# importZL/semantic_segmentation

Hardware: AMD Instinct MI355X
Metric: images/sec (fwd+bwd) U-Net 256x256 bs=32 per GPU (higher is better)
Workload: dtype f16; 1 GPU; unet.UNet(1,2) 256x256 fwd+bwd, CE+Dice loss, batch 32/GPU (BASELINE configs[1]); global_batch=32, parallelism=dp1, dice=per-rank

## Files before the change

### include/gsseg.h

```cpp
#ifndef GSSEG_H
#define GSSEG_H

#include <stdint.h>

#ifdef __cplusplus
extern "C" {
#endif

#define GS_ABI_VERSION 52

enum GsDtype { GS_F16 = 0, GS_BF16 = 1 };
enum GsStatus { GS_OK = 0, GS_EINVAL = -1, GS_ELAUNCH = -2, GS_EUNSUPPORTED = -3 };
enum GsAct { GS_ACT_NONE = 0, GS_ACT_RELU = 1, GS_ACT_LEAKY02 = 2, GS_ACT_TANH = 3 };

#define GS_MAX_TAPS 64

typedef struct GsConvGeom {
    int32_t N, IH, IW, Cin, in_pix_stride, in_coff;
    int32_t OHg, OWg, Cout;
    int32_t OH, OW, out_pix_stride, out_coff;
    int32_t isy, isx, osy, osx, ooy, oox;
    int32_t ntaps;
    int32_t tap_dy[GS_MAX_TAPS], tap_dx[GS_MAX_TAPS];
    int32_t tap_w[GS_MAX_TAPS];
    int32_t Dg, Din, Dout, isz, osz, ooz;
    int32_t tap_dz[GS_MAX_TAPS];
} GsConvGeom;

const char* gs_last_error(void);
int gs_abi_version(void);

int gs_conv_igemm_mtiles(const GsConvGeom* g);
int64_t gs_conv_igemm_workspace_floats(void);
int gs_conv_igemm(const GsConvGeom* g, const void* x, const void* w, void* y, const float* bias,
                  float* bn_partials, int act, int dtype, float* splitk_ws, int64_t splitk_ws_floats, void* stream);
int gs_conv_igemm_batch(int n, const GsConvGeom* const* g, const void* x, const void* const* w, void* y, const float* bias,
                        float* const* bn_partials, int act, int dtype, float* splitk_ws, int64_t splitk_ws_floats,
                        void* stream);

int gs_upconv2x2_fwd(const void* x, const void* w, const float* bias, void* y, int N, int D, int IH, int IW, int Cin,
                     int in_pix_stride, int in_coff, int Cout, int Dout, int OH, int OW, int out_pix_stride,
                     int out_coff, int ooz, int ooy, int oox, int act, int dtype, void* stream);

int gs_upconv2x2_dgrad(const void* dy, const void* wd, void* dx, int N, int IH, int IW, int Cin, int Cout, int OH, int OW,
                       int dy_pix_stride, int dy_coff, int ooy, int oox, int dx_pix_stride, int dx_coff, int dtype,
                       void* stream);

int gs_conv3x3_mtiles(int N, int H, int W, int Cout);
int gs_conv3x3_stat_rows(int N, int H, int W, int Cin, int Cout, int pair);
int gs_conv3x3_set_kernel_form(int form);
int gs_set_persistent_grid(int blocks);
int gs_get_persistent_grid(void);
int gs_conv3x3(const void* x, const void* w, void* y, const float* bias, float* bn_partials, int N, int H, int W,
               int Cin, int in_pix_stride, int in_coff, int Cout, int out_pix_stride, int out_coff,
               const int32_t* tap_dy, const int32_t* tap_dx, int act, int dtype, void* stream);

int gs_conv3x3_wgrad(const void* x, const void* dy, float* dw, int N, int H, int W, int Cin, int in_pix_stride,
                     int in_coff, int Cout, int out_pix_stride, int out_coff, int dtype, void* stream);

int gs_conv_wgrad(const GsConvGeom* g, const void* x, const void* dy, float* dw, int dtype, void* stream);
int gs_conv_wgrad_single_pass(const GsConvGeom* g);
int gs_conv_wgrad_assign(const GsConvGeom* g, const void* x, const void* dy, float* dw, int dtype, void* stream);
int gs_conv_wgrad_parts(const GsConvGeom* g);
int64_t gs_conv_wgrad_ws_floats(const GsConvGeom* g);
int gs_conv_wgrad_slabs(const GsConvGeom* g, const void* x, const void* dy, float* ws, int dtype, void* stream);
int gs_conv_wgrad_slabs_batch(int n, const GsConvGeom* const* g, const void* x, const void* dy, float* ws, int dtype,
                              void* stream);

int gs_conv_smallcin_mtiles(int N, int OH, int OW);
int gs_conv_smallcin_fwd(const float* x, const float* w, const float* bias, void* y, float* bn_partials,
                         int N, int Cin, int IH, int IW, int Cout, int OH, int OW, int k, int stride, int pad,
                         int act, int dtype, void* stream);
int64_t gs_conv_direct_wgrad_ws_floats(int N, int OH, int OW, int Cin, int Cout, int k);

int gs_stem_stats(const float* x, const float* w, float* bn_partials, float* tap_sums, int N, int H, int W, void* stream);
int gs_stem_fwd_bn(const float* x, const float* w, const float* bn_scale, const float* bn_shift, int act, void* z, int N,
                   int H, int W, int dtype, void* stream);
int gs_stem_bwd_tiles(int N, int H, int W);
int gs_stem_bwd_onepass(const float* x, const void* z, const void* dz, int dz_stride, int dz_coff, int act,
                        float* s1_partials, float* ws, int N, int H, int W, int dtype, void* stream);
int gs_stem_bwd_finalize(const float* ws, const float* s1_partials, const float* tap_sums, const float* w,
                         const float* scale, const float* mean, const float* invstd, int train_stats, float gscale, float* dw,
                         float* dgamma, float* dbeta, int N, int H, int W, void* stream);

int gs_stem_bn_bwd_wgrad(const void* y, const void* dz, int dz_stride, int dz_coff, const float* x, const float* scale,
                         const float* shift, const float* mean, const float* invstd, const float* c1, const float* c2,
                         int act, float* dw, float* ws, int N, int H, int W, float gscale, int dtype, void* stream);

int gs_conv_smallcin_wgrad(const float* x, const void* dy, float* dw, float* ws, int N, int Cin, int IH, int IW,
                           int Cout, int OH, int OW, int k, int stride, int pad, float gscale, int dtype, void* stream);
int gs_conv_smallcin_dgrad(const void* dy, const float* w, float* dx, int N, int Cin, int IH, int IW, int Cout,
// ... 252 lines not shown
```

### semantic_segmentation_amd/_lib.py

```python
from __future__ import annotations

import ctypes
import os
import subprocess
from ctypes import POINTER, c_char_p, c_double, c_float, c_int, c_int32, c_int64, c_void_p

_HERE = os.path.dirname(os.path.abspath(__file__))
LIB_PATH = os.environ.get("GSSEG_LIB", os.path.join(_HERE, "libgsseg_hip.so"))
CSRC = os.path.join(_HERE, "csrc")

GS_F16, GS_BF16 = 0, 1
ACT_NONE, ACT_RELU, ACT_LEAKY02, ACT_TANH = 0, 1, 2, 3
GS_MAX_TAPS = 64
ABI_VERSION = 52


class GsConvGeom(ctypes.Structure):
    _fields_ = [(n, c_int32) for n in (
        "N", "IH", "IW", "Cin", "in_pix_stride", "in_coff", "OHg", "OWg", "Cout", "OH", "OW",
        "out_pix_stride", "out_coff", "isy", "isx", "osy", "osx", "ooy", "oox", "ntaps")] + [
        ("tap_dy", c_int32 * GS_MAX_TAPS), ("tap_dx", c_int32 * GS_MAX_TAPS), ("tap_w", c_int32 * GS_MAX_TAPS)] + [
        (n, c_int32) for n in ("Dg", "Din", "Dout", "isz", "osz", "ooz")] + [("tap_dz", c_int32 * GS_MAX_TAPS)]


class GsPackDesc(ctypes.Structure):
    _fields_ = [("w", c_void_p), ("w_fwd", c_void_p), ("w_dgrad", c_void_p)] + [
        (n, c_int32) for n in ("Cout", "Cin", "taps", "transposed")]


GS_SEG_MAX = 4


class GsSegPackDesc(ctypes.Structure):
    _fields_ = [("w", c_void_p), ("pack", c_void_p)] + [(n, c_int32) for n in ("Cout", "Cin", "taps", "transposed", "nseg")] + [
        ("kind", c_int32 * GS_SEG_MAX), ("ci0", c_int32 * GS_SEG_MAX), ("len", c_int32 * GS_SEG_MAX)]


class GsQ8PackDesc(ctypes.Structure):
    _fields_ = [("w", c_void_p), ("pack", c_void_p), ("wexp", c_void_p)] + [(n, c_int32) for n in ("Cout", "Cin", "taps")]


_P, _F = c_void_p, c_void_p
PROTOTYPES = {
    "gs_last_error": (c_char_p, []),
    "gs_abi_version": (c_int, []),
    "gs_conv_igemm_mtiles": (c_int, [POINTER(GsConvGeom)]),
    "gs_conv3x3_stat_rows": (c_int, [c_int] * 6),
    "gs_upconv2x2_wgrad_parts": (c_int, [c_int] * 5),
    "gs_upconv2x2_wgrad_ws_floats": (c_int64, [c_int] * 5),
    "gs_upconv2x2_wgrad_slabs": (c_int, [_P, _P, _F] + [c_int] * 14 + [c_void_p]),
    "gs_set_persistent_grid": (c_int, [c_int]),
    "gs_get_persistent_grid": (c_int, []),
    "gs_conv_igemm": (c_int, [POINTER(GsConvGeom), _P, _P, _P, _F, _F, c_int, c_int, _F, c_int64, c_void_p]),
    "gs_conv_igemm_workspace_floats": (c_int64, []),
    "gs_conv_igemm_batch": (c_int, [c_int, POINTER(POINTER(GsConvGeom)), _P, POINTER(c_void_p), _P, _F, POINTER(c_void_p),
                                    c_int, c_int, _F, c_int64, c_void_p]),
    "gs_upconv2x2_fwd": (c_int, [_P, _P, _F, _P] + [c_int] * 18 + [c_void_p]),
    "gs_upconv2x2_dgrad": (c_int, [c_void_p, c_void_p, c_void_p] + [c_int] * 14 + [c_void_p]),
    "gs_conv3x3_mtiles": (c_int, [c_int, c_int, c_int, c_int]),
    "gs_conv3x3_set_kernel_form": (c_int, [c_int]),
    "gs_conv3d_3x3x3_mtiles": (c_int, [c_int] * 5),
    "gs_conv3d_3x3x3": (c_int, [_P, _P, _P, _F, _F] + [c_int] * 10 + [POINTER(c_int32)] * 3 + [c_int, c_int, c_void_p]),
    "gs_conv3d_3x3x3_wgrad_ws_floats": (c_int64, [c_int] * 6),
    "gs_conv3d_3x3x3_wgrad_parts": (c_int, [c_int] * 6),
    "gs_conv3d_3x3x3_wgrad_slabs": (c_int, [_P, _P, _F] + [c_int] * 11 + [c_void_p]),
    "gs_conv3d_3x3x3_wgrad": (c_int, [_P, _P, _F] + [c_int] * 11 + [c_void_p]),
    "gs_upsample2x_bilinear_fwd": (c_int, [_P, _P] + [c_int] * 13 + [c_void_p]),
    "gs_upsample2x_bilinear_bwd": (c_int, [_P, _P] + [c_int] * 13 + [c_void_p]),
    "gs_affine_warp": (c_int, [_F, _F, _F, c_int, c_int, c_int, c_int, c_float, c_void_p]),
    "gs_optim_chunk_elems": (c_int, []),
    "gs_optim_rmsprop": (c_int, [_P] * 7 + [c_int] + [c_float] * 6 + [c_void_p]),
    "gs_optim_adam": (c_int, [_P] * 7 + [c_int, _P] + [c_float] * 5 + [c_void_p]),
    "gs_conv3x3": (c_int, [_P, _P, _P, _F, _F] + [c_int] * 9 + [POINTER(c_int32), POINTER(c_int32), c_int, c_int, c_void_p]),
    "gs_conv3x3_wgrad": (c_int, [_P, _P, _F] + [c_int] * 10 + [c_void_p]),
    "gs_conv3x3_wgrad_ws_floats": (c_int64, [c_int] * 5),
    "gs_conv3x3_wgrad_parts": (c_int, [c_int] * 5),
    "gs_conv3x3_wgrad_slabs": (c_int, [_P, _P, _F] + [c_int] * 10 + [c_void_p]),
    "gs_wgrad_reduce_unpack": (c_int, [_F, c_int, _F, c_int, c_int, c_int, c_int, c_float, c_void_p]),
    "gs_conv_wgrad": (c_int, [POINTER(GsConvGeom), _P, _P, _F, c_int, c_void_p]),
    "gs_conv_wgrad_assign": (c_int, [POINTER(GsConvGeom), _P, _P, _F, c_int, c_void_p]),
    "gs_conv_wgrad_single_pass": (c_int, [POINTER(GsConvGeom)]),
    "gs_conv_wgrad_parts": (c_int, [POINTER(GsConvGeom)]),
    "gs_conv_wgrad_ws_floats": (c_int64, [POINTER(GsConvGeom)]),
    "gs_conv_wgrad_slabs": (c_int, [POINTER(GsConvGeom), _P, _P, _F, c_int, c_void_p]),
    "gs_conv_wgrad_slabs_batch": (c_int, [c_int, POINTER(POINTER(GsConvGeom)), _P, _P, _F, c_int, c_void_p]),
    "gs_conv_smallcin_mtiles": (c_int, [c_int, c_int, c_int]),
    "gs_conv_smallcin_fwd": (c_int, [_F, _F, _F, _P, _F] + [c_int] * 12 + [c_void_p]),
    "gs_conv_direct_wgrad_ws_floats": (c_int64, [c_int] * 6),
    "gs_conv_smallcin_wgrad": (c_int, [_F, _P, _F, _F] + [c_int] * 10 + [c_float, c_int, c_void_p]),
    "gs_conv_smallcin_dgrad": (c_int, [_P, _F, _F] + [c_int] * 10 + [c_float, c_int, c_void_p]),
    "gs_conv_smallcout_fwd": (c_int, [_P, _F, _F, _F] + [c_int] * 11 + [c_void_p]),
    "gs_conv_smallcout_bwd": (c_int, [_P, _F, _F, _P, _F, _F, _F] + [c_int] * 10 + [c_float, c_int, c_void_p]),
    "gs_bn_partials_floats": (c_int64, [c_int, c_int]),
    "gs_bn_finalize": (c_int, [_F, c_int, c_int, c_double, _F, _F, _F, _F, c_float, c_float, _F, _F, _F, _F, c_void_p]),
    "gs_bn_eval_coeffs": (c_int, [c_int, _F, _F, _F, _F, c_float, _F, _F, _F, _F, c_void_p]),
    "gs_bn_act_apply": (c_int, [_P, _F, _F, c_int, _P, c_int, c_int, _P, _P, c_float] + [c_int] * 5 + [c_void_p]),
    "gs_bn_bwd_tiles": (c_int, [c_int, c_int, c_int]),
    "gs_bn_bwd_tiles_used": (c_int, [c_int, c_int, c_int, c_int]),
    "gs_bn_act_bwd_reduce": (c_int, [_P, _P, c_int, c_int, _P, _P, c_int, _P, c_float, _F, _F, _F, _F, c_int, _F]
                             + [c_int] * 5 + [c_void_p]),
    "gs_bn_bwd_coeffs": (c_int, [_F, c_int, c_int, c_double, c_float, _F, _F, _F, _F, c_void_p]),
    "gs_bn_act_bwd_apply": (c_int, [_P, _P, c_int, c_int, _P, _P, c_int, _P, c_float, _F, _F, _F, _F, _F, _F, c_int,
                                    c_int, _P]
                            + [c_int] * 5 + [c_void_p]),
    "gs_maxpool3d_fwd": (c_int, [_P, c_int, c_int, _P] + [c_int] * 6 + [c_void_p]),
    "gs_maxpool2x2_fwd": (c_int, [_P, c_int, c_int, _P] + [c_int] * 5 + [c_void_p]),
    "gs_maxpool2x2_fwd_pair": (c_int, [_P, _P, c_int, _P, _P, c_int] + [c_int] * 5 + [c_void_p]),
# ... 126 lines not shown
```

### semantic_segmentation_amd/csrc/wgrad3x3.hip

```cpp
#include <stdlib.h>

#include "common.hpp"

namespace {

struct W3Args {
    const unsigned short* x;
    const unsigned short* dy;
    float* dw;
    int N, H, W, Cin, in_stride, in_coff, Cout, out_stride, out_coff;
    int tiles_x, tiles_y, npatches, ncob, ncib, ksplit, pps;
    int D, dz;
    int64_t slab_stride;
};

constexpr int W3_LDR = 96;
constexpr int W3_BM = 128;

template <int DT, int TW>
__global__ __launch_bounds__(256, 2) void wgrad3x3_kernel(const W3Args a) {
    typedef typename Elem<DT>::V8 V8;
    constexpr int TH = W3_BM / TW;
    constexpr int HWD = TW + 2, HHT = TH + 2, HP = HWD * HHT;
    constexpr int DY_EL = W3_BM * W3_LDR, H_EL = HP * W3_LDR;
    constexpr int HCH = (HP * 8 + 255) / 256;
    constexpr int TWS = (TW == 32) ? 5 : 4;
    constexpr unsigned OOB = 0xFFFFFFFFu;
    __shared__ __attribute__((aligned(16))) unsigned short smem[DY_EL + H_EL];
    unsigned short* dyt = smem;
    unsigned short* halo = smem + DY_EL;

    const int t = threadIdx.x, lane = t & 63, wave = t >> 6;
    const int wm = wave >> 1, wn = wave & 1;
// ... 97 lines not shown
                const int hrow = (py + tap / 3) * HWD + px0 + tap % 3;
                const V8 bf = tr_read8<DT>(b_base + hrow * W3_LDR, b_base + (hrow + 4) * W3_LDR);
                acc[tap] = Elem<DT>::mfma32(af, bf, acc[tap]);
            }
        }
    }

    const int l31 = lane & 31, h = lane >> 5;
    const int ci = ci0 + wn * 32 + l31;
    if (ci < a.Cin) {
#pragma unroll
        for (int tap = 0; tap < 9; ++tap)
#pragma unroll
            for (int r = 0; r < 16; ++r) {
                const int co = co0 + wm * 32 + (r & 3) + 8 * (r >> 2) + 4 * h;
                if (co < a.Cout) {
                    float* q = a.dw + ((int64_t)tap * a.Cout + co) * a.Cin + ci;
                    if (a.slab_stride > 0) q[(int64_t)ks * a.slab_stride] = acc[tap][r];
                    else atomicAdd(q, acc[tap][r]);
                }
            }
    }
}


__device__ __forceinline__ void w3_dma_piece16(const __amdgpu_buffer_rsrc_t& rs, unsigned char* dst, unsigned voff) {
    const unsigned lds_addr = (unsigned)(size_t)(LDS_AS void*)dst;
    unsigned keep;
    asm volatile("s_mov_b32 %0, m0\n\ts_mov_b32 m0, %1\n\ts_nop 0\n\tbuffer_load_dwordx4 %2, %3, 0 offen lds\n\ts_mov_b32 m0, %0"
                 : "=&s"(keep) : "s"(lds_addr), "v"(voff), "s"(rs) : "memory");
}
__device__ __forceinline__ void w3_opaque(unsigned& x) { asm volatile("" : "+v"(x)); }

template <int DT>
__global__ __launch_bounds__(512, 1) void wgrad3x3_dma_kernel(const W3Args a) {
    typedef typename Elem<DT>::V8 V8;
    constexpr int TW = 32, TH = 8, TWS = 5, BM = 256;
    constexpr int HWD = TW + 2, HHT = TH + 2, HP = HWD * HHT;
    static_assert(BM / 8 == 4 * 8, "32 dY pieces: four per wave");
    constexpr int HJ = 6;
    constexpr int HPC = (HP + 7) / 8;
    constexpr int DY_B = BM * 128, HALO_B = (HPC + 1) * 1024;
    constexpr int HALO_OFF = 2 * DY_B;
    constexpr unsigned VOOB = 0x80000000u;
    static_assert(HPC + 1 <= HJ * 8 && 2 * (DY_B + HALO_B) <= 160 * 1024, "LDS budget");
    static_assert(4 * 9 * 16 * 64 * 4 <= 2 * (DY_B + HALO_B), "final in-block reduction overlays the stage buffers");
    __shared__ __attribute__((aligned(1024))) unsigned char smem[2 * (DY_B + HALO_B)];

    const int t = threadIdx.x, lane = t & 63;
    const int wave = __builtin_amdgcn_readfirstlane(t >> 6);
    const int grp = wave >> 2;
    const int wm = (wave >> 1) & 1, wn = wave & 1;
    int bid;
    {
        const int nwg = gridDim.x, q = nwg >> 3, r = nwg & 7, xcd = blockIdx.x & 7;
        bid = ((xcd < r) ? xcd * (q + 1) : r * (q + 1) + (xcd - r) * q) + (blockIdx.x >> 3);
    }
    const int cob = bid % a.ncob; bid /= a.ncob;
    const int cib = bid % a.ncib; bid /= a.ncib;
    const int ks = bid;
    const int co0 = cob * 64, ci0 = cib * 64;
    const int p_begin = ks * a.pps;
    const int p_end = min(a.npatches, p_begin + a.pps);
    if (p_begin >= p_end) return;

    const unsigned x_img_bytes = (unsigned)a.H * a.W * a.in_stride * 2u;
    const unsigned dy_img_bytes = (unsigned)a.H * a.W * a.out_stride * 2u;
// ... 64 lines not shown

    f32x16 acc[9];
#pragma unroll
    for (int i = 0; i < 9; ++i)
#pragma unroll
        for (int r = 0; r < 16; ++r) acc[i][r] = 0.f;

    const int G = lane >> 4, q = (lane & 15) >> 2, pp = lane & 3;
    const int krow = 8 * (G >> 1) + q;
    const int chn = 16 * (G & 1) + 4 * pp;
    unsigned a_base0 = (unsigned)((grp * 16 + krow) * 128 + (((wm ^ ((q >> 1) & 1)) * 32 + chn) * 2));
    unsigned b_base0[4];
#pragma unroll
    for (int c4 = 0; c4 < 4; ++c4)
        b_base0[c4] = (unsigned)(HALO_OFF + (grp * 16 + krow) * 128 + (((wn ^ (((c4 + q) >> 1) & 1)) * 32 + chn) * 2));

    {
        const Pf f0 = prep_patch(true);
#pragma unroll
        for (int k = 0; k < 4 + HJ; ++k) issue_piece(f0, k, 0u);
    }
    for (int patch = p_begin; patch < p_end; ++patch) {
        asm volatile("s_waitcnt vmcnt(0)" ::: "memory");
        __builtin_amdgcn_s_barrier();
        asm volatile("" ::: "memory");
        const unsigned buf = (unsigned)(patch - p_begin) & 1u;
        const bool more = patch + 1 < p_end;
        const Pf pf = prep_patch(more);
        unsigned ab = a_base0 + buf * DY_B, bb[4];
#pragma unroll
        for (int c4 = 0; c4 < 4; ++c4) { bb[c4] = b_base0[c4] + buf * HALO_B; w3_opaque(bb[c4]); }
        w3_opaque(ab);
        const LDS_AS unsigned char* lds = (const LDS_AS unsigned char*)smem;
        constexpr int PD = 3;
        V8 afr[2], bfr[PD + 1];
        auto load_a = [&](int s, V8& dst) __attribute__((always_inline)) {
            dst = tr_read8<DT>((const LDS_AS unsigned short*)(lds + ab + s * 32 * 128),
                               (const LDS_AS unsigned short*)(lds + ab + (s * 32 + 4) * 128));
        };
        auto load_b = [&](int step, V8& dst) __attribute__((always_inline)) {
            const int s = step / 9, tap = step - 9 * s;
            const int C = (s + tap / 3) * HWD + tap % 3;
            dst = tr_read8<DT>((const LDS_AS unsigned short*)(lds + bb[C & 3] + C * 128),
                               (const LDS_AS unsigned short*)(lds + bb[C & 3] + (C + 4) * 128));
        };
        load_a(0, afr[0]);
#pragma unroll
        for (int i = 0; i < PD; ++i) load_b(i, bfr[i]);
#pragma unroll
        for (int step = 0; step < 72; ++step) {
            const int s = step / 9, tap = step - 9 * s;
            if (step + PD < 72) load_b(step + PD, bfr[(step + PD) % (PD + 1)]);
            if (tap == 4 && s + 1 < 8) load_a(s + 1, afr[(s + 1) & 1]);
#if !defined(GS_W3_ABLATE) || GS_W3_ABLATE != 1
            if (s < 4 && (tap == 1 || tap == 4 || tap == 7) && 3 * s + tap / 3 < 4 + HJ) issue_piece(pf, 3 * s + tap / 3, buf ^ 1u);
#endif
#if !defined(GS_W3_ABLATE) || GS_W3_ABLATE != 2
            acc[tap] = Elem<DT>::mfma32(afr[s & 1], bfr[step % (PD + 1)], acc[tap]);
#endif
            __builtin_amdgcn_sched_group_barrier(0x008, 1, 0);
            __builtin_amdgcn_sched_group_barrier(0x100, 4, 0);
            __builtin_amdgcn_sched_barrier(0);
        }
    }
    asm volatile("s_waitcnt vmcnt(0)" ::: "memory");
    __syncthreads();
    float* xch = reinterpret_cast<float*>(smem) + (wave & 3) * (9 * 16 * 64) + lane;
    if (grp == 1) {
#pragma unroll
        for (int tap = 0; tap < 9; ++tap)
#pragma unroll
            for (int r = 0; r < 16; ++r) xch[(tap * 16 + r) * 64] = acc[tap][r];
    }
    __syncthreads();
    if (grp == 1) return;
    const int l31 = lane & 31, h = lane >> 5;
    const int ci = ci0 + wn * 32 + l31;
#pragma unroll
    for (int tap = 0; tap < 9; ++tap)
#pragma unroll
        for (int r = 0; r < 16; ++r) {
            const float v = acc[tap][r] + xch[(tap * 16 + r) * 64];
            const int co = co0 + wm * 32 + (r & 3) + 8 * (r >> 2) + 4 * h;
            if (ci < a.Cin && co < a.Cout) {
                float* qd = a.dw + ((int64_t)tap * a.Cout + co) * a.Cin + ci;
                if (a.slab_stride > 0) qd[(int64_t)ks * a.slab_stride] = v;
                else atomicAdd(qd, v);
            }
        }
}

template <int DT>
__global__ __launch_bounds__(512, 1) void wgrad3x3_dma128_kernel(const W3Args a) {
    typedef typename Elem<DT>::V8 V8;
    constexpr int TW = 32, TH = 4, TWS = 5, BM = 128;
    constexpr int HWD = TW + 2, HHT = TH + 2, HP = HWD * HHT;
    constexpr int DJ = 4;
    constexpr int HPC = (HP + 7) / 8;
    constexpr int HJ = 4;
    constexpr int IMG_B = BM * 128;
    constexpr int DY_B = 2 * IMG_B, HALO_B = (HPC + 1) * 1024;
    constexpr int HALO_OFF = 2 * DY_B;
    constexpr unsigned VOOB = 0x80000000u;
    static_assert(HPC + 1 <= HJ * 8 && 2 * (DY_B + HALO_B) <= 160 * 1024, "LDS budget");
    __shared__ __attribute__((aligned(1024))) unsigned char smem[2 * (DY_B + HALO_B)];

    const int t = threadIdx.x, lane = t & 63;
    const int wave = __builtin_amdgcn_readfirstlane(t >> 6);
    const int wmm = wave >> 1, wn = wave & 1;
    int bid;
    {
        const int nwg = gridDim.x, q = nwg >> 3, r = nwg & 7, xcd = blockIdx.x & 7;
        bid = ((xcd < r) ? xcd * (q + 1) : r * (q + 1) + (xcd - r) * q) + (blockIdx.x >> 3);
    }
    const int cob = bid % a.ncob; bid /= a.ncob;
    const int cib = bid % a.ncib; bid /= a.ncib;
    const int ks = bid;
    const int co0 = cob * 128, ci0 = cib * 64;
    const int p_begin = ks * a.pps;
    const int p_end = min(a.npatches, p_begin + a.pps);
    if (p_begin >= p_end) return;

    const unsigned x_img_bytes = (unsigned)a.H * a.W * a.in_stride * 2u;
    const unsigned dy_img_bytes = (unsigned)a.H * a.W * a.out_stride * 2u;
    const int drow = lane >> 3;
// ... 67 lines not shown

    f32x16 acc[9];
#pragma unroll
    for (int i = 0; i < 9; ++i)
#pragma unroll
        for (int r = 0; r < 16; ++r) acc[i][r] = 0.f;

    const int G = lane >> 4, q = (lane & 15) >> 2, pp = lane & 3;
    const int krow = 8 * (G >> 1) + q;
    const int chn = 16 * (G & 1) + 4 * pp;
    unsigned a_base0 = (unsigned)((wmm >> 1) * IMG_B + krow * 128 + ((((wmm & 1) ^ ((q >> 1) & 1)) * 32 + chn) * 2));
    unsigned b_base0[4];
#pragma unroll
    for (int c4 = 0; c4 < 4; ++c4)
        b_base0[c4] = (unsigned)(HALO_OFF + krow * 128 + (((wn ^ (((c4 + q) >> 1) & 1)) * 32 + chn) * 2));

    {
        const Pf f0 = prep_patch(true);
#pragma unroll
        for (int k = 0; k < DJ + HJ; ++k) issue_piece(f0, k, 0u);
    }
    for (int patch = p_begin; patch < p_end; ++patch) {
        asm volatile("s_waitcnt vmcnt(0)" ::: "memory");
        __builtin_amdgcn_s_barrier();
        asm volatile("" ::: "memory");
        const unsigned buf = (unsigned)(patch - p_begin) & 1u;
        const bool more = patch + 1 < p_end;
        const Pf pf = prep_patch(more);
        unsigned ab = a_base0 + buf * DY_B, bb[4];
#pragma unroll
        for (int c4 = 0; c4 < 4; ++c4) { bb[c4] = b_base0[c4] + buf * HALO_B; w3_opaque(bb[c4]); }
        w3_opaque(ab);
        const LDS_AS unsigned char* lds = (const LDS_AS unsigned char*)smem;
        constexpr int PD = 3;
        V8 afr[2], bfr[PD + 1];
        auto load_a = [&](int sg, V8& dst) __attribute__((always_inline)) {
            dst = tr_read8<DT>((const LDS_AS unsigned short*)(lds + ab + sg * 16 * 128),
                               (const LDS_AS unsigned short*)(lds + ab + (sg * 16 + 4) * 128));
        };
        auto load_b = [&](int step, V8& dst) __attribute__((always_inline)) {
            const int sg = step / 9, tap = step - 9 * sg;
            const int s = sg >> 1, g = sg & 1;
            const int C = (s + tap / 3) * HWD + tap % 3 + 16 * g;
            dst = tr_read8<DT>((const LDS_AS unsigned short*)(lds + bb[C & 3] + C * 128),
                               (const LDS_AS unsigned short*)(lds + bb[C & 3] + (C + 4) * 128));
        };
        load_a(0, afr[0]);
#pragma unroll
        for (int i = 0; i < PD; ++i) load_b(i, bfr[i]);
#pragma unroll
        for (int step = 0; step < 72; ++step) {
            const int sg = step / 9, tap = step - 9 * sg;
            if (step + PD < 72) load_b(step + PD, bfr[(step + PD) % (PD + 1)]);
            if (tap == 4 && sg + 1 < 8) load_a(sg + 1, afr[(sg + 1) & 1]);
            if (sg < 3 && (tap == 1 || tap == 4 || tap == 7) && 3 * sg + tap / 3 < DJ + HJ) issue_piece(pf, 3 * sg + tap / 3, buf ^ 1u);
            acc[tap] = Elem<DT>::mfma32(afr[sg & 1], bfr[step % (PD + 1)], acc[tap]);
            __builtin_amdgcn_sched_group_barrier(0x008, 1, 0);
            __builtin_amdgcn_sched_group_barrier(0x100, 4, 0);
            __builtin_amdgcn_sched_barrier(0);
        }
    }
    asm volatile("s_waitcnt vmcnt(0)" ::: "memory");
    const int l31 = lane & 31, h = lane >> 5;
    const int ci = ci0 + wn * 32 + l31;
#pragma unroll
    for (int tap = 0; tap < 9; ++tap)
#pragma unroll
        for (int r = 0; r < 16; ++r) {
            const int co = co0 + wmm * 32 + (r & 3) + 8 * (r >> 2) + 4 * h;
            if (ci < a.Cin && co < a.Cout) {
                float* qd = a.dw + ((int64_t)tap * a.Cout + co) * a.Cin + ci;
                if (a.slab_stride > 0) qd[(int64_t)ks * a.slab_stride] = acc[tap][r];
                else atomicAdd(qd, acc[tap][r]);
            }
        }
}
}

static bool w3_use_dma(int W) {
    static const int env = getenv("GSSEG_W3_DMA") ? atoi(getenv("GSSEG_W3_DMA")) : 1;
    return env != 0 && W >= 24;
}

static bool w3_use_co128(int W, int Cout) {
    static const int env = getenv("GSSEG_W3_CO128") ? atoi(getenv("GSSEG_W3_CO128")) : 1;
    return env != 0 && w3_use_dma(W) && Cout % 128 == 0;
}

static int w3_ksplit(int N, int H, int W, int Cin, int Cout, int* pps_out, int* npatches_out, bool dma) {
    const bool co128 = dma && w3_use_co128(W, Cout);
    const int tw = (W >= 24) ? 32 : 16, th = co128 ? 4 : (dma ? 8 : W3_BM / tw);
    const int npatches = N * cdiv(W, tw) * cdiv(H, th);
    const int pairs = cdiv(Cout, co128 ? 128 : 64) * cdiv(Cin, 64);
    static const int target_env = getenv("GSSEG_W3_GRID") ? atoi(getenv("GSSEG_W3_GRID")) : 0;
    const int target = target_env > 0 ? target_env : (dma ? gs_get_persistent_grid() : 2 * gs_get_persistent_grid());
    static const int min_pps_env = getenv("GSSEG_W3_MINPPS") ? atoi(getenv("GSSEG_W3_MINPPS")) : 4;
    const int min_pps = (dma && !co128) ? (min_pps_env + 1) / 2 : min_pps_env;
    int ksplit = target / pairs;
    if (ksplit > npatches / min_pps) ksplit = npatches / min_pps;
    if (ksplit < 1) ksplit = 1;
    const int pps = cdiv(npatches, ksplit);
    if (pps_out) *pps_out = pps;
    if (npatches_out) *npatches_out = npatches;
    return cdiv(npatches, pps);
}

static int wgrad3x3_launch(const void* x, const void* dy, float* dw, int N, int H, int W, int Cin,
                           int in_pix_stride, int in_coff, int Cout, int out_pix_stride, int out_coff, int dtype,
                           void* stream, int D, int dz, int64_t slab_stride = 0) {
    GS_CHECK_ARG(x && dy && dw, "gs_conv3x3_wgrad: null pointer");
    GS_CHECK_ARG(N > 0 && H > 0 && W > 0 && Cin > 0 && Cin % 8 == 0 && Cout > 0 && Cout % 8 == 0, "gs_conv3x3_wgrad: bad dims");
    GS_CHECK_ARG(in_pix_stride >= in_coff + Cin && in_pix_stride % 8 == 0 && in_coff % 8 == 0, "gs_conv3x3_wgrad: bad x stride");
    GS_CHECK_ARG(out_pix_stride >= out_coff + Cout && out_pix_stride % 8 == 0 && out_coff % 8 == 0, "gs_conv3x3_wgrad: bad dy stride");
    GS_CHECK_ARG((int64_t)H * W * in_pix_stride * 2 < 4294967000LL && (int64_t)H * W * out_pix_stride * 2 < 4294967000LL,
                 "gs_conv3x3_wgrad: one image must stay below 4 GiB (32-bit buffer offsets)");
    GS_CHECK_ARG(dtype == GS_F16 || dtype == GS_BF16, "gs_conv3x3_wgrad: bad dtype");
    W3Args a;
    a.x = (const unsigned short*)x; a.dy = (const unsigned short*)dy; a.dw = dw;
    a.N = N; a.H = H; a.W = W; a.Cin = Cin; a.in_stride = in_pix_stride; a.in_coff = in_coff;
    a.Cout = Cout; a.out_stride = out_pix_stride; a.out_coff = out_coff;
    a.D = D; a.dz = dz; a.slab_stride = slab_stride;
    const bool dma = w3_use_dma(W);
    const bool co128 = dma && w3_use_co128(W, Cout);
    const int tw = (W >= 24) ? 32 : 16, th = co128 ? 4 : (dma ? 8 : W3_BM / tw);
    a.tiles_x = cdiv(W, tw); a.tiles_y = cdiv(H, th);
    a.npatches = N * a.tiles_x * a.tiles_y;
    a.ncob = cdiv(Cout, co128 ? 128 : 64); a.ncib = cdiv(Cin, 64);
    const int pairs = a.ncob * a.ncib;
    {
        int pps = 0, np = 0;
        a.ksplit = w3_ksplit(N, H, W, Cin, Cout, &pps, &np, dma);
        a.pps = pps;
    }
    hipStream_t s = (hipStream_t)stream;
    if (dma) {
        dim3 dgrid(pairs * a.ksplit);
        if (co128) {
            if (dtype == GS_F16) wgrad3x3_dma128_kernel<GS_F16><<<dgrid, 512, 0, s>>>(a);
            else wgrad3x3_dma128_kernel<GS_BF16><<<dgrid, 512, 0, s>>>(a);
        } else if (dtype == GS_F16) wgrad3x3_dma_kernel<GS_F16><<<dgrid, 512, 0, s>>>(a);
        else wgrad3x3_dma_kernel<GS_BF16><<<dgrid, 512, 0, s>>>(a);
        GS_CHECK_LAUNCH("gs_conv3x3_wgrad");
        return GS_OK;
    }
    dim3 grid(pairs * a.ksplit), block(256);
    if (dtype == GS_F16) {
        if (tw == 32) wgrad3x3_kernel<GS_F16, 32><<<grid, block, 0, s>>>(a);
        else wgrad3x3_kernel<GS_F16, 16><<<grid, block, 0, s>>>(a);
    } else {
        if (tw == 32) wgrad3x3_kernel<GS_BF16, 32><<<grid, block, 0, s>>>(a);
        else wgrad3x3_kernel<GS_BF16, 16><<<grid, block, 0, s>>>(a);
    }
    GS_CHECK_LAUNCH("gs_conv3x3_wgrad");
    return GS_OK;
}

extern "C" int gs_conv3x3_wgrad(const void* x, const void* dy, float* dw, int N, int H, int W, int Cin,
                                int in_pix_stride, int in_coff, int Cout, int out_pix_stride, int out_coff, int dtype,
                                void* stream) {
    return wgrad3x3_launch(x, dy, dw, N, H, W, Cin, in_pix_stride, in_coff, Cout, out_pix_stride, out_coff, dtype, stream, 1, 0);
}

extern "C" int gs_conv3d_3x3x3_wgrad(const void* x, const void* dy, float* dw, int NB, int D, int H, int W, int Cin,
                                     int in_pix_stride, int in_coff, int Cout, int out_pix_stride, int out_coff, int dtype,
                                     void* stream) {
    GS_CHECK_ARG(NB > 0 && D > 0 && dw, "gs_conv3d_3x3x3_wgrad: bad arguments");
    for (int kd = 0; kd < 3; ++kd) {
        if (D == 1 && kd != 1) continue;
        int rc = wgrad3x3_launch(x, dy, dw + (int64_t)kd * 9 * Cout * Cin, NB * D, H, W, Cin, in_pix_stride, in_coff, Cout,
                                 out_pix_stride, out_coff, dtype, stream, D, kd - 1);
        if (rc) return rc;
    }
    return GS_OK;
}
// ... 156 lines not shown
```

### semantic_segmentation_amd/ops.py

```python
from __future__ import annotations

import collections
import ctypes
import os
from typing import List, Optional, Sequence, Tuple

import torch

from . import _lib
from ._lib import ACT_NONE, GS_BF16, GS_F16, GsConvGeom

DTYPES = {"f16": (GS_F16, torch.float16), "bf16": (GS_BF16, torch.bfloat16)}


def dt_code(t: torch.Tensor) -> int:
    if t.dtype == torch.float16:
        return GS_F16
    if t.dtype == torch.bfloat16:
        return GS_BF16
    raise TypeError(f"expected a float16/bfloat16 tensor, got {t.dtype}")


def _p(t: Optional[torch.Tensor]):
    return None if t is None else t.data_ptr()
# ... 227 lines not shown
    _lib.call("gs_conv_igemm_batch", n, garr, _p(x), warr, _p(y), _p(bias), parr, act, dt_code(x), _p(ws),
              ws.numel() if ws is not None else 0, stream)
    if ev is not None:
        TIMER.stop("igemm_fwd", ev, sum(_geom_flops(g) for g in geoms), sum(_geom_bytes(g) for g in geoms))


TAPS3_FWD = [(ky - 1, kx - 1) for ky in range(3) for kx in range(3)]
TAPS3_DGRAD = [(1 - ky, 1 - kx) for ky in range(3) for kx in range(3)]
USE_HALO_CONV = os.environ.get("GSSEG_CONV3X3", "halo") != "generic"


def conv3x3_mtiles(N, H, W, Cout) -> int:
    return _lib.load().gs_conv3x3_mtiles(N, H, W, Cout)


def conv3x3_stat_rows(N, H, W, Cin, Cout, pair=False) -> int:
    return int(_lib.load().gs_conv3x3_stat_rows(N, H, W, Cin, Cout, 2 if pair == "q" else (1 if pair else 0)))


def conv3d3_stat_rows(NB, D, H, W, Cin, Cout) -> int:
    return conv3x3_stat_rows(NB * D, H, W, Cin, Cout)


def set_persistent_grid(blocks: int = 0) -> None:
    _lib.call("gs_set_persistent_grid", int(blocks))


def get_persistent_grid() -> int:
    return int(_lib.load().gs_get_persistent_grid())


def conv3x3_set_kernel_form(form: int = -1) -> None:
    _lib.call("gs_conv3x3_set_kernel_form", int(form))


def conv3x3(x, w, y, N, H, W, Cin, Cout, taps=TAPS3_FWD, bias=None, bn_partials=None, act=ACT_NONE,
            in_stride=None, in_coff=0, out_stride=None, out_coff=0):
    _dev(x)
    _f32(bias, "bias"); _f32(bn_partials, "bn_partials")
    if not (x.dtype == w.dtype == y.dtype):
        raise TypeError("conv3x3: x, w, y must share one 16-bit dtype")
    if bn_partials is not None and bn_partials.numel() < bn_partials_numel(conv3x3_stat_rows(N, H, W, Cin, Cout), Cout):
        raise ValueError("conv3x3: bn_partials too small (conv3x3_stat_rows rows of [2][Cout])")
    dy, dx = _tap_arrays(taps)
    ev = TIMER.start() if TIMER is not None else None
    _lib.call("gs_conv3x3", _p(x), _p(w), _p(y), _p(bias), _p(bn_partials), N, H, W, Cin,
              Cin if in_stride is None else in_stride, in_coff, Cout, Cout if out_stride is None else out_stride,
              out_coff, dy, dx, act, dt_code(x), _stream())
    if ev is not None:
        TIMER.stop("conv3x3_halo", ev, 2.0 * N * H * W * Cout * 9 * Cin,
                   2.0 * (N * H * W * (Cin + Cout) + 9 * Cin * Cout))


def conv3x3_wgrad(x, dy, dw, N, H, W, Cin, Cout, in_stride=None, in_coff=0, out_stride=None, out_coff=0):
    _dev(x)
    _f32(dw, "dw")
    if x.dtype != dy.dtype:
        raise TypeError("conv3x3_wgrad: x and dy must share one 16-bit dtype")
    if dw.numel() < 9 * Cout * Cin:
        raise ValueError("conv3x3_wgrad: dw too small")
    ev = TIMER.start() if TIMER is not None else None
    _lib.call("gs_conv3x3_wgrad", _p(x), _p(dy), _p(dw), N, H, W, Cin, Cin if in_stride is None else in_stride,
              in_coff, Cout, Cout if out_stride is None else out_stride, out_coff, dt_code(x), _stream())
    if ev is not None:
        TIMER.stop("wgrad3x3_halo", ev, 2.0 * N * H * W * Cout * 9 * Cin,
                   2.0 * N * H * W * (Cin + Cout) + 4.0 * 9 * Cin * Cout)
# ... 1100 lines not shown
```

Baseline: 2132 images/sec.

## Reuse each input-row LDS fragment across all three ky taps in wgrad3x3 DMA kernels

Adds a REUSE variant of the DMA 3x3 weight-gradient kernels. The loop now walks halo input rows and column taps, loads each B fragment from LDS once, and feeds it into up to three MFMAs (one per ky) against cached dy fragments. The old form loaded the B fragment separately for every output-row/tap pair. This cuts LDS transpose reads, at the cost of keeping more A fragments live in registers and changing the prefetch-issue schedule. By default it is enabled only for the Cout%128 path, and an env var and a setter allow switching forms.

```diff
diff --git a/include/gsseg.h b/include/gsseg.h
--- a/include/gsseg.h
+++ b/include/gsseg.h
@@ -7,7 +7,7 @@
 extern "C" {
 #endif
 
-#define GS_ABI_VERSION 52
+#define GS_ABI_VERSION 53
 
 enum GsDtype { GS_F16 = 0, GS_BF16 = 1 };
 enum GsStatus { GS_OK = 0, GS_EINVAL = -1, GS_ELAUNCH = -2, GS_EUNSUPPORTED = -3 };
@@ -57,6 +57,7 @@
 
 int gs_conv3x3_wgrad(const void* x, const void* dy, float* dw, int N, int H, int W, int Cin, int in_pix_stride,
                      int in_coff, int Cout, int out_pix_stride, int out_coff, int dtype, void* stream);
+int gs_conv3x3_wgrad_set_form(int form);
 
 int gs_conv_wgrad(const GsConvGeom* g, const void* x, const void* dy, float* dw, int dtype, void* stream);
 int gs_conv_wgrad_single_pass(const GsConvGeom* g);
diff --git a/semantic_segmentation_amd/_lib.py b/semantic_segmentation_amd/_lib.py
--- a/semantic_segmentation_amd/_lib.py
+++ b/semantic_segmentation_amd/_lib.py
@@ -12,7 +12,7 @@
 GS_F16, GS_BF16 = 0, 1
 ACT_NONE, ACT_RELU, ACT_LEAKY02, ACT_TANH = 0, 1, 2, 3
 GS_MAX_TAPS = 64
-ABI_VERSION = 52
+ABI_VERSION = 53
 
 
 class GsConvGeom(ctypes.Structure):
@@ -73,6 +73,7 @@
     "gs_optim_adam": (c_int, [_P] * 7 + [c_int, _P] + [c_float] * 5 + [c_void_p]),
     "gs_conv3x3": (c_int, [_P, _P, _P, _F, _F] + [c_int] * 9 + [POINTER(c_int32), POINTER(c_int32), c_int, c_int, c_void_p]),
     "gs_conv3x3_wgrad": (c_int, [_P, _P, _F] + [c_int] * 10 + [c_void_p]),
+    "gs_conv3x3_wgrad_set_form": (c_int, [c_int]),
     "gs_conv3x3_wgrad_ws_floats": (c_int64, [c_int] * 5),
     "gs_conv3x3_wgrad_parts": (c_int, [c_int] * 5),
     "gs_conv3x3_wgrad_slabs": (c_int, [_P, _P, _F] + [c_int] * 10 + [c_void_p]),
diff --git a/semantic_segmentation_amd/csrc/wgrad3x3.hip b/semantic_segmentation_amd/csrc/wgrad3x3.hip
--- a/semantic_segmentation_amd/csrc/wgrad3x3.hip
+++ b/semantic_segmentation_amd/csrc/wgrad3x3.hip
@@ -1,4 +1,6 @@
 #include <stdlib.h>
+
+#include <atomic>
 
 #include "common.hpp"
 
@@ -162,7 +164,7 @@
 }
 __device__ __forceinline__ void w3_opaque(unsigned& x) { asm volatile("" : "+v"(x)); }
 
-template <int DT>
+template <int DT, bool REUSE>
 __global__ __launch_bounds__(512, 1) void wgrad3x3_dma_kernel(const W3Args a) {
     typedef typename Elem<DT>::V8 V8;
     constexpr int TW = 32, TH = 8, TWS = 5, BM = 256;
@@ -293,35 +295,74 @@
         for (int c4 = 0; c4 < 4; ++c4) { bb[c4] = b_base0[c4] + buf * HALO_B; w3_opaque(bb[c4]); }
         w3_opaque(ab);
         const LDS_AS unsigned char* lds = (const LDS_AS unsigned char*)smem;
-        constexpr int PD = 3;
-        V8 afr[2], bfr[PD + 1];
-        auto load_a = [&](int s, V8& dst) __attribute__((always_inline)) {
-            dst = tr_read8<DT>((const LDS_AS unsigned short*)(lds + ab + s * 32 * 128),
-                               (const LDS_AS unsigned short*)(lds + ab + (s * 32 + 4) * 128));
-        };
-        auto load_b = [&](int step, V8& dst) __attribute__((always_inline)) {
-            const int s = step / 9, tap = step - 9 * s;
-            const int C = (s + tap / 3) * HWD + tap % 3;
-            dst = tr_read8<DT>((const LDS_AS unsigned short*)(lds + bb[C & 3] + C * 128),
-                               (const LDS_AS unsigned short*)(lds + bb[C & 3] + (C + 4) * 128));
-        };
-        load_a(0, afr[0]);
-#pragma unroll
-        for (int i = 0; i < PD; ++i) load_b(i, bfr[i]);
-#pragma unroll
-        for (int step = 0; step < 72; ++step) {
-            const int s = step / 9, tap = step - 9 * s;
-            if (step + PD < 72) load_b(step + PD, bfr[(step + PD) % (PD + 1)]);
-            if (tap == 4 && s + 1 < 8) load_a(s + 1, afr[(s + 1) & 1]);
+        if constexpr (REUSE) {
+            constexpr int NU = HHT * 3;
+            constexpr int PD = 3;
+            constexpr int PC0 = 0, PCS = 1;
+            V8 afr[4], bfr[PD + 1];
+            auto load_a = [&](int s, V8& dst) __attribute__((always_inline)) {
+                dst = tr_read8<DT>((const LDS_AS unsigned short*)(lds + ab + s * 32 * 128),
+                                   (const LDS_AS unsigned short*)(lds + ab + (s * 32 + 4) * 128));
+            };
+            auto load_b = [&](int u, V8& dst) __attribute__((always_inline)) {
+                const int C = (u / 3) * HWD + u % 3;
+                dst = tr_read8<DT>((const LDS_AS unsigned short*)(lds + bb[C & 3] + C * 128),
+                                   (const LDS_AS unsigned short*)(lds + bb[C & 3] + (C + 4) * 128));
+            };
+            load_a(0, afr[0]);
+#pragma unroll
+            for (int i = 0; i < PD; ++i) load_b(i, bfr[i]);
+#pragma unroll
+            for (int u = 0; u < NU; ++u) {
+                const int r = u / 3, kx = u - 3 * r;
+                if (u + PD < NU) load_b(u + PD, bfr[(u + PD) % (PD + 1)]);
+                if (kx == 0 && r + 1 < TH) load_a(r + 1, afr[(r + 1) & 3]);
 #if !defined(GS_W3_ABLATE) || GS_W3_ABLATE != 1
-            if (s < 4 && (tap == 1 || tap == 4 || tap == 7) && 3 * s + tap / 3 < 4 + HJ) issue_piece(pf, 3 * s + tap / 3, buf ^ 1u);
+                if (u >= PC0 && (u - PC0) % PCS == 0 && (u - PC0) / PCS < 4 + HJ) issue_piece(pf, (u - PC0) / PCS, buf ^ 1u);
 #endif
 #if !defined(GS_W3_ABLATE) || GS_W3_ABLATE != 2
-            acc[tap] = Elem<DT>::mfma32(afr[s & 1], bfr[step % (PD + 1)], acc[tap]);
+#pragma unroll
+                for (int ky = 0; ky < 3; ++ky) {
+                    const int s = r - ky;
+                    if (s >= 0 && s < TH) acc[3 * ky + kx] = Elem<DT>::mfma32(afr[s & 3], bfr[u % (PD + 1)], acc[3 * ky + kx]);
+                }
 #endif
-            __builtin_amdgcn_sched_group_barrier(0x008, 1, 0);
-            __builtin_amdgcn_sched_group_barrier(0x100, 4, 0);
-            __builtin_amdgcn_sched_barrier(0);
+                __builtin_amdgcn_sched_group_barrier(0x008, 1, 0);
+                __builtin_amdgcn_sched_group_barrier(0x100, 4, 0);
+                __builtin_amdgcn_sched_group_barrier(0x008, 2, 0);
+                __builtin_amdgcn_sched_barrier(0);
+            }
+        } else {
+            constexpr int PD = 3;
+            V8 afr[2], bfr[PD + 1];
+            auto load_a = [&](int s, V8& dst) __attribute__((always_inline)) {
+                dst = tr_read8<DT>((const LDS_AS unsigned short*)(lds + ab + s * 32 * 128),
+                                   (const LDS_AS unsigned short*)(lds + ab + (s * 32 + 4) * 128));
+            };
+            auto load_b = [&](int step, V8& dst) __attribute__((always_inline)) {
+                const int s = step / 9, tap = step - 9 * s;
+                const int C = (s + tap / 3) * HWD + tap % 3;
+                dst = tr_read8<DT>((const LDS_AS unsigned short*)(lds + bb[C & 3] + C * 128),
+                                   (const LDS_AS unsigned short*)(lds + bb[C & 3] + (C + 4) * 128));
+            };
+            load_a(0, afr[0]);
+#pragma unroll
+            for (int i = 0; i < PD; ++i) load_b(i, bfr[i]);
+#pragma unroll
+            for (int step = 0; step < 72; ++step) {
+                const int s = step / 9, tap = step - 9 * s;
+                if (step + PD < 72) load_b(step + PD, bfr[(step + PD) % (PD + 1)]);
+                if (tap == 4 && s + 1 < 8) load_a(s + 1, afr[(s + 1) & 1]);
+#if !defined(GS_W3_ABLATE) || GS_W3_ABLATE != 1
+                if (s < 4 && (tap == 1 || tap == 4 || tap == 7) && 3 * s + tap / 3 < 4 + HJ) issue_piece(pf, 3 * s + tap / 3, buf ^ 1u);
+#endif
+#if !defined(GS_W3_ABLATE) || GS_W3_ABLATE != 2
+                acc[tap] = Elem<DT>::mfma32(afr[s & 1], bfr[step % (PD + 1)], acc[tap]);
+#endif
+                __builtin_amdgcn_sched_group_barrier(0x008, 1, 0);
+                __builtin_amdgcn_sched_group_barrier(0x100, 4, 0);
+                __builtin_amdgcn_sched_barrier(0);
+            }
         }
     }
     asm volatile("s_waitcnt vmcnt(0)" ::: "memory");
@@ -351,7 +392,7 @@
         }
 }
 
-template <int DT>
+template <int DT, bool REUSE>
 __global__ __launch_bounds__(512, 1) void wgrad3x3_dma128_kernel(const W3Args a) {
     typedef typename Elem<DT>::V8 V8;
     constexpr int TW = 32, TH = 4, TWS = 5, BM = 128;
@@ -485,32 +526,69 @@
         for (int c4 = 0; c4 < 4; ++c4) { bb[c4] = b_base0[c4] + buf * HALO_B; w3_opaque(bb[c4]); }
         w3_opaque(ab);
         const LDS_AS unsigned char* lds = (const LDS_AS unsigned char*)smem;
-        constexpr int PD = 3;
-        V8 afr[2], bfr[PD + 1];
-        auto load_a = [&](int sg, V8& dst) __attribute__((always_inline)) {
-            dst = tr_read8<DT>((const LDS_AS unsigned short*)(lds + ab + sg * 16 * 128),
-                               (const LDS_AS unsigned short*)(lds + ab + (sg * 16 + 4) * 128));
-        };
-        auto load_b = [&](int step, V8& dst) __attribute__((always_inline)) {
-            const int sg = step / 9, tap = step - 9 * sg;
-            const int s = sg >> 1, g = sg & 1;
-            const int C = (s + tap / 3) * HWD + tap % 3 + 16 * g;
-            dst = tr_read8<DT>((const LDS_AS unsigned short*)(lds + bb[C & 3] + C * 128),
-                               (const LDS_AS unsigned short*)(lds + bb[C & 3] + (C + 4) * 128));
-        };
-        load_a(0, afr[0]);
-#pragma unroll
-        for (int i = 0; i < PD; ++i) load_b(i, bfr[i]);
-#pragma unroll
-        for (int step = 0; step < 72; ++step) {
-            const int sg = step / 9, tap = step - 9 * sg;
-            if (step + PD < 72) load_b(step + PD, bfr[(step + PD) % (PD + 1)]);
-            if (tap == 4 && sg + 1 < 8) load_a(sg + 1, afr[(sg + 1) & 1]);
-            if (sg < 3 && (tap == 1 || tap == 4 || tap == 7) && 3 * sg + tap / 3 < DJ + HJ) issue_piece(pf, 3 * sg + tap / 3, buf ^ 1u);
-            acc[tap] = Elem<DT>::mfma32(afr[sg & 1], bfr[step % (PD + 1)], acc[tap]);
-            __builtin_amdgcn_sched_group_barrier(0x008, 1, 0);
-            __builtin_amdgcn_sched_group_barrier(0x100, 4, 0);
-            __builtin_amdgcn_sched_barrier(0);
+        if constexpr (REUSE) {
+            constexpr int NU = HHT * 6;
+            constexpr int PD = 3;
+            constexpr int PC0 = 0, PCS = 1;
+            V8 afr[2 * TH], bfr[PD + 1];
+            auto load_a = [&](int sg, V8& dst) __attribute__((always_inline)) {
+                dst = tr_read8<DT>((const LDS_AS unsigned short*)(lds + ab + sg * 16 * 128),
+                                   (const LDS_AS unsigned short*)(lds + ab + (sg * 16 + 4) * 128));
+            };
+            auto load_b = [&](int u, V8& dst) __attribute__((always_inline)) {
+                const int r = u / 6, g = (u / 3) & 1, kx = u % 3;
+                const int C = r * HWD + kx + 16 * g;
+                dst = tr_read8<DT>((const LDS_AS unsigned short*)(lds + bb[C & 3] + C * 128),
+                                   (const LDS_AS unsigned short*)(lds + bb[C & 3] + (C + 4) * 128));
+            };
+            load_a(0, afr[0]);
+            load_a(1, afr[1]);
+#pragma unroll
+            for (int i = 0; i < PD; ++i) load_b(i, bfr[i]);
+#pragma unroll
+            for (int u = 0; u < NU; ++u) {
+                const int r = u / 6, g = (u / 3) & 1, kx = u % 3;
+                if (u + PD < NU) load_b(u + PD, bfr[(u + PD) % (PD + 1)]);
+                if (g == 0 && kx < 2 && r + 1 < TH) load_a(2 * (r + 1) + kx, afr[2 * (r + 1) + kx]);
+                if (u >= PC0 && (u - PC0) % PCS == 0 && (u - PC0) / PCS < DJ + HJ) issue_piece(pf, (u - PC0) / PCS, buf ^ 1u);
+#pragma unroll
+                for (int ky = 0; ky < 3; ++ky) {
+                    const int s = r - ky;
+                    if (s >= 0 && s < TH) acc[3 * ky + kx] = Elem<DT>::mfma32(afr[2 * s + g], bfr[u % (PD + 1)], acc[3 * ky + kx]);
+                }
+                __builtin_amdgcn_sched_group_barrier(0x008, 1, 0);
+                __builtin_amdgcn_sched_group_barrier(0x100, 4, 0);
+                __builtin_amdgcn_sched_group_barrier(0x008, 2, 0);
+                __builtin_amdgcn_sched_barrier(0);
+            }
+        } else {
+            constexpr int PD = 3;
+            V8 afr[2], bfr[PD + 1];
+            auto load_a = [&](int sg, V8& dst) __attribute__((always_inline)) {
+                dst = tr_read8<DT>((const LDS_AS unsigned short*)(lds + ab + sg * 16 * 128),
+                                   (const LDS_AS unsigned short*)(lds + ab + (sg * 16 + 4) * 128));
+            };
+            auto load_b = [&](int step, V8& dst) __attribute__((always_inline)) {
+                const int sg = step / 9, tap = step - 9 * sg;
+                const int s = sg >> 1, g = sg & 1;
+                const int C = (s + tap / 3) * HWD + tap % 3 + 16 * g;
+                dst = tr_read8<DT>((const LDS_AS unsigned short*)(lds + bb[C & 3] + C * 128),
+                                   (const LDS_AS unsigned short*)(lds + bb[C & 3] + (C + 4) * 128));
+            };
+            load_a(0, afr[0]);
+#pragma unroll
+            for (int i = 0; i < PD; ++i) load_b(i, bfr[i]);
+#pragma unroll
+            for (int step = 0; step < 72; ++step) {
+                const int sg = step / 9, tap = step - 9 * sg;
+                if (step + PD < 72) load_b(step + PD, bfr[(step + PD) % (PD + 1)]);
+                if (tap == 4 && sg + 1 < 8) load_a(sg + 1, afr[(sg + 1) & 1]);
+                if (sg < 3 && (tap == 1 || tap == 4 || tap == 7) && 3 * sg + tap / 3 < DJ + HJ) issue_piece(pf, 3 * sg + tap / 3, buf ^ 1u);
+                acc[tap] = Elem<DT>::mfma32(afr[sg & 1], bfr[step % (PD + 1)], acc[tap]);
+                __builtin_amdgcn_sched_group_barrier(0x008, 1, 0);
+                __builtin_amdgcn_sched_group_barrier(0x100, 4, 0);
+                __builtin_amdgcn_sched_barrier(0);
+            }
         }
     }
     asm volatile("s_waitcnt vmcnt(0)" ::: "memory");
@@ -538,6 +616,14 @@
 static bool w3_use_co128(int W, int Cout) {
     static const int env = getenv("GSSEG_W3_CO128") ? atoi(getenv("GSSEG_W3_CO128")) : 1;
     return env != 0 && w3_use_dma(W) && Cout % 128 == 0;
+}
+
+static std::atomic<int> w3_reuse_form{getenv("GSSEG_W3_REUSE") ? (atoi(getenv("GSSEG_W3_REUSE")) != 0 ? 1 : 0) : -1};
+
+extern "C" int gs_conv3x3_wgrad_set_form(int form) {
+    GS_CHECK_ARG(form == 0 || form == 1, "gs_conv3x3_wgrad_set_form: form must be 0 (X fragment read once per ky) or 1 (read once, reused)");
+    w3_reuse_form.store(form, std::memory_order_relaxed);
+    return GS_OK;
 }
 
 static int w3_ksplit(int N, int H, int W, int Cin, int Cout, int* pps_out, int* npatches_out, bool dma) {
@@ -588,11 +674,23 @@
     hipStream_t s = (hipStream_t)stream;
     if (dma) {
         dim3 dgrid(pairs * a.ksplit);
+        const int form = w3_reuse_form.load(std::memory_order_relaxed);
+        const bool reuse = form < 0 ? co128 : form != 0;
         if (co128) {
-            if (dtype == GS_F16) wgrad3x3_dma128_kernel<GS_F16><<<dgrid, 512, 0, s>>>(a);
-            else wgrad3x3_dma128_kernel<GS_BF16><<<dgrid, 512, 0, s>>>(a);
-        } else if (dtype == GS_F16) wgrad3x3_dma_kernel<GS_F16><<<dgrid, 512, 0, s>>>(a);
-        else wgrad3x3_dma_kernel<GS_BF16><<<dgrid, 512, 0, s>>>(a);
+            if (dtype == GS_F16) {
+                if (reuse) wgrad3x3_dma128_kernel<GS_F16, true><<<dgrid, 512, 0, s>>>(a);
+                else wgrad3x3_dma128_kernel<GS_F16, false><<<dgrid, 512, 0, s>>>(a);
+            } else {
+                if (reuse) wgrad3x3_dma128_kernel<GS_BF16, true><<<dgrid, 512, 0, s>>>(a);
+                else wgrad3x3_dma128_kernel<GS_BF16, false><<<dgrid, 512, 0, s>>>(a);
+            }
+        } else if (dtype == GS_F16) {
+            if (reuse) wgrad3x3_dma_kernel<GS_F16, true><<<dgrid, 512, 0, s>>>(a);
+            else wgrad3x3_dma_kernel<GS_F16, false><<<dgrid, 512, 0, s>>>(a);
+        } else {
+            if (reuse) wgrad3x3_dma_kernel<GS_BF16, true><<<dgrid, 512, 0, s>>>(a);
+            else wgrad3x3_dma_kernel<GS_BF16, false><<<dgrid, 512, 0, s>>>(a);
+        }
         GS_CHECK_LAUNCH("gs_conv3x3_wgrad");
         return GS_OK;
     }
diff --git a/semantic_segmentation_amd/ops.py b/semantic_segmentation_amd/ops.py
--- a/semantic_segmentation_amd/ops.py
+++ b/semantic_segmentation_amd/ops.py
@@ -283,6 +283,10 @@
 
 def conv3x3_set_kernel_form(form: int = -1) -> None:
     _lib.call("gs_conv3x3_set_kernel_form", int(form))
+
+
+def conv3x3_wgrad_set_form(form: int = 1) -> None:
+    _lib.call("gs_conv3x3_wgrad_set_form", int(form))
 
 
 def conv3x3(x, w, y, N, H, W, Cin, Cout, taps=TAPS3_FWD, bias=None, bn_partials=None, act=ACT_NONE,
```

New measurement: 2140 images/sec (median of 6 runs). No clear change (+0.4%).
